# Luigi940260/orb-slam2-optimized

Measured on AMD Instinct MI355X. Metric: RANSAC hypotheses/sec (EPnP relocalization batch, 2k corrs x 64 candidates), higher is better.
Workload: dtype f64; 1 GPU; config 2 reloc_pnp: candidates x correspondences, iterate(300), exhaustive (40% inliers); candidates=64, candidates_per_gpu=64, correspondences=2000, hypotheses_per_candidate=300, params=SetRansacParameters(0.99,10,300,4,0.5,5.991)

## Files before the change

### orb-slam2-optimized_amd/csrc/kernels.hip

```cpp
#include <hip/hip_runtime.h>
#include <climits>

#ifndef RSC_REFINE_STAMPS
#define RSC_REFINE_STAMPS 0
#endif
namespace rsc {
__device__ uint64_t g_refine_stamps[64][24];
}
#ifndef RSC_SOLVE_STAMPS
#define RSC_SOLVE_STAMPS 0
#endif
namespace rsc {
__device__ uint64_t g_solve_stamps[3][4096][8];
}
#if RSC_SOLVE_STAMPS
#define RSC_JSVD_STAMP(k, j)                                                                           \
    do {                                                                                               \
        if (blockIdx.x < 4096 && (threadIdx.x & 63) == 0 && blockDim.x == 64) {                       \
            ::rsc::g_solve_stamps[2][blockIdx.x][j] = wall_clock64();                                  \
            ::rsc::g_solve_stamps[2][blockIdx.x][3] = (k);                                             \
        }                                                                                              \
    } while (0)
#define RSC_SOLVE_STAMP(st, k)                                                                         \
    do {                                                                                               \
        if (blockIdx.x < 4096 && (threadIdx.x & 63) == 0) ::rsc::g_solve_stamps[st][blockIdx.x][k] = wall_clock64(); \
    } while (0)
#endif
#include "rsc_core.h"
#include "rsc_epnp.h"
#include "rsc_sim3.h"
#if RSC_REFINE_STAMPS
#define RSC_EIG_PHASE(k)                                                                               \
    do {                                                                                               \
        if (blockIdx.x < 64 && threadIdx.x == 0) ::rsc::g_refine_stamps[blockIdx.x][8 + (k)] = wall_clock64(); \
    } while (0)
#endif
#include "rsc_quad.h"
#include "rsc_math.h"
#include "rsc_kernels.h"

namespace rsc {

template <int NS>
__global__ __launch_bounds__(64) void pnp_eig_group_kernel(const DevPnP* __restrict__ probs,
                                                          const LaunchProb* __restrict__ lps,
                                                          const int2* __restrict__ wg_table,
                                                          const uint32_t* __restrict__ rng_T,
                                                          double* __restrict__ stage, int32_t* __restrict__ samples) {
    __shared__ __attribute__((aligned(16))) double smem[kEigHyps * kQuadRegion];
    pnp_eig_group_body<NS, 99, kEigLanes, kEigHyps>(probs, lps, wg_table, rng_T, stage, samples, smem);
}

template <int NS>
__global__ __launch_bounds__(128 * kSplitUnits) __attribute__((amdgpu_waves_per_eu(2))) void pnp_eig_split_kernel(
    const DevPnP* __restrict__ probs, const LaunchProb* __restrict__ lps, const int2* __restrict__ wg_table,
    int nwg_table, const uint32_t* __restrict__ rng_T, double* __restrict__ stage, int32_t* __restrict__ samples,
    unsigned* fault) {
    __shared__ __attribute__((aligned(16))) double smem[kSplitHyps * kQuadRegion];
    __shared__ __attribute__((aligned(16))) double dsub[kSplitHyps * kSplitDsub];
    __shared__ int pub[kSplitUnits], ack[kSplitUnits];
    pnp_eig_split_body<NS>(probs, lps, wg_table, nwg_table, rng_T, stage, samples, smem, dsub, pub, ack, fault);
}

template <int NS>
__global__ __launch_bounds__(64) void pnp_betas_kernel(const DevPnP* __restrict__ probs,
                                                       const LaunchProb* __restrict__ lps,
                                                       const int2* __restrict__ wg_table, int ngroups,
                                                       const double* __restrict__ stage,
                                                       const int32_t* __restrict__ samples,
                                                       double* __restrict__ berr, float* __restrict__ bpose,
                                                       size_t hcap, int hb) {
    __shared__ __attribute__((aligned(16))) double smem[kBetasWaveSmemDoubles];
    pnp_betas_wave_body<NS>(probs, lps, wg_table, ngroups, hb, stage, samples, berr, bpose, hcap, smem);
}

typedef float rsc_f2 __attribute__((ext_vector_type(2)));
__device__ __forceinline__ void pnp_inlier2(const float (&R)[9], const float (&t)[3], double fx, double fy, double cx,
                                            double cy, rsc_f2 X, rsc_f2 Y, rsc_f2 Z, rsc_f2 u, rsc_f2 v, rsc_f2 maxErr,
                                            bool& in0, bool& in1, bool& ok) {
    const rsc_f2 Xc = (R[0] * X + (R[1] * Y + R[2] * Z)) + t[0];
    const rsc_f2 Yc = (R[3] * X + (R[4] * Y + R[5] * Z)) + t[1];
    const rsc_f2 Zc = (R[6] * X + (R[7] * Y + R[8] * Z)) + t[2];
    const rsc_f2 r0 = {__builtin_amdgcn_rcpf(Zc.x), __builtin_amdgcn_rcpf(Zc.y)};
    const rsc_f2 e = __builtin_elementwise_fma(-Zc, r0, (rsc_f2){1.0f, 1.0f});
    const rsc_f2 iz = __builtin_elementwise_fma(e, r0, r0);
    const float a0 = fabsf(Zc.x), a1 = fabsf(Zc.y);
    ok = ok & (a0 >= 0x1p-126f) & (a0 <= 0x1p125f) & (a1 >= 0x1p-126f) & (a1 <= 0x1p125f);
    const rsc_f2 ue = {(float)(cx + fx * (double)Xc.x * (double)iz.x), (float)(cx + fx * (double)Xc.y * (double)iz.y)};
    const rsc_f2 ve = {(float)(cy + fy * (double)Yc.x * (double)iz.x), (float)(cy + fy * (double)Yc.y * (double)iz.y)};
    const rsc_f2 du = ue - u, dv = ve - v;
    const rsc_f2 e2 = du * du + dv * dv;
    in0 = e2.x < maxErr.x;
    in1 = e2.y < maxErr.y;
}

template <int PPT>
__global__ __launch_bounds__(256) void pnp_scan_kernel(const DevPnP* __restrict__ probs,
                                                       const LaunchProb* __restrict__ lps,
                                                       const int4* __restrict__ wg_table,
                                                       const double* __restrict__ berr,
                                                       const float* __restrict__ bpose, size_t hcap,
                                                       float* __restrict__ poses,
                                                       int32_t* __restrict__ counts,
                                                       int32_t* __restrict__ counts_dev,
                                                       uint64_t* __restrict__ masks, int mask_words,
                                                       int32_t* __restrict__ qual) {
    constexpr int B = PPT <= 8 ? 64 : 512 / PPT;
    __shared__ int wave_cnt[4][B];
    __shared__ uint64_t mbuf[B][4][PPT];
    const int tid = threadIdx.x, lane = tid & 63, wave = tid >> 6;
    const int4 wt = wg_table[blockIdx.x];
    const LaunchProb& lp = lps[wt.x];
    const DevPnP& P = probs[lp.prob];
    const double fx = P.fx, fy = P.fy, cx = P.cx, cy = P.cy;
    const size_t rec0 = (size_t)(lp.out0 + wt.y);
    double e0 = 0.0, e1 = 0.0, e2 = 0.0;
    if (lane < wt.z) {
        e0 = berr[rec0 + lane];
        e1 = berr[hcap + rec0 + lane];
        e2 = berr[2 * hcap + rec0 + lane];
    }
    float X[PPT], Y[PPT], Z[PPT], U[PPT], V[PPT], E[PPT];
    RSC_UNROLL for (int s = 0; s < PPT; ++s) {
        const int i = s * 256 + tid;
        if (i < P.n) {
            const float4 p = P.pts[i];
            const float2 q = P.uv[i];
            X[s] = p.x; Y[s] = p.y; Z[s] = p.z; E[s] = p.w * P.th2; U[s] = q.x; V[s] = q.y;
        } else {
            X[s] = 0.f; Y[s] = 0.f; Z[s] = 1.f; E[s] = -1.f; U[s] = 0.f; V[s] = 0.f;
        }
    }
    int best = 0;
    {
        double be = e0;
        if (e1 < be) { be = e1; best = 1; }
        if (e2 < be) { be = e2; best = 2; }
    }
    const uint64_t pick1 = __ballot(best == 1), pick2 = __ballot(best == 2);
    auto pose_of = [&](int j) {
        const size_t apx = (size_t)((pick1 >> j) & 1u) + 2 * (size_t)((pick2 >> j) & 1u);
        return bpose + (apx * hcap + rec0 + (size_t)j) * 12;
    };
    for (int w = tid; w < wt.z * 12; w += 256) {
        const int hj = w / 12, k = w - 12 * hj;
        poses[(rec0 + hj) * 12 + k] = pose_of(hj)[k];
    }
    const float* pp = pose_of(0);
    float Rn[9], tn[3];
    RSC_UNROLL for (int k = 0; k < 9; ++k) Rn[k] = pp[k];
    RSC_UNROLL for (int k = 0; k < 3; ++k) tn[k] = pp[9 + k];
    for (int j = 0; j < wt.z; ++j) {
        float R[9], t[3];
        RSC_UNROLL for (int k = 0; k < 9; ++k) R[k] = Rn[k];
        RSC_UNROLL for (int k = 0; k < 3; ++k) t[k] = tn[k];
        if (j + 1 < wt.z) {
            pp = pose_of(j + 1);
            RSC_UNROLL for (int k = 0; k < 9; ++k) Rn[k] = pp[k];
            RSC_UNROLL for (int k = 0; k < 3; ++k) tn[k] = pp[9 + k];
        }
        uint64_t b[PPT];
        if constexpr (PPT >= 2) {
            bool ok = true;
            RSC_UNROLL for (int s = 0; s < PPT; s += 2) {
                bool i0, i1;
                pnp_inlier2(R, t, fx, fy, cx, cy, (rsc_f2){X[s], X[s + 1]}, (rsc_f2){Y[s], Y[s + 1]},
                            (rsc_f2){Z[s], Z[s + 1]}, (rsc_f2){U[s], U[s + 1]}, (rsc_f2){V[s], V[s + 1]},
                            (rsc_f2){E[s], E[s + 1]}, i0, i1, ok);
                b[s] = __ballot(i0);
                b[s + 1] = __ballot(i1);
            }
            if (__builtin_expect(__any(!ok), 0)) {
                RSC_UNROLL for (int s = 0; s < PPT; ++s)
                    b[s] = __ballot(pnp_inlier(R, t, fx, fy, cx, cy, X[s], Y[s], Z[s], U[s], V[s], E[s]));
            }
        } else {
            RSC_UNROLL for (int s = 0; s < PPT; ++s)
                b[s] = __ballot(pnp_inlier(R, t, fx, fy, cx, cy, X[s], Y[s], Z[s], U[s], V[s], E[s]));
        }
        int cnt = 0;
        uint64_t mine = 0;
        RSC_UNROLL for (int s = 0; s < PPT; ++s) {
            cnt += __popcll(b[s]);
            mine = (lane == s) ? b[s] : mine;
        }
        const int jb = j % B;
        if (lane < PPT) mbuf[jb][wave][lane] = mine;
        if (lane == 0) wave_cnt[wave][jb] = cnt;
        if (jb == B - 1 || j == wt.z - 1) {
            __syncthreads();
            const int base = j - jb;
            if (tid <= jb) {
                const int c = wave_cnt[0][tid] + wave_cnt[1][tid] + wave_cnt[2][tid] + wave_cnt[3][tid];
                counts[lp.out0 + wt.y + base + tid] = c;
                if (counts_dev) counts_dev[lp.out0 + wt.y + base + tid] = c;
                if (c >= lp.min_inliers) qual[wt.x] = 1;
                wave_cnt[0][tid] = c;
            }
            __syncthreads();
            if (masks) {
                for (int w = tid; w < (jb + 1) * 4 * PPT; w += 256) {
                    const int hb = w / (4 * PPT), r = w - hb * (4 * PPT), s = r >> 2, wv = r & 3;
                    if (wave_cnt[0][hb] >= lp.min_inliers)
                        masks[(size_t)(lp.out0 + wt.y + base + hb) * mask_words + r] = mbuf[hb][wv][s];
                }
            }
            __syncthreads();
        }
    }
}

__device__ __forceinline__ void wave_lds_sync() {
    __builtin_amdgcn_fence(__ATOMIC_RELEASE, "wavefront");
    __builtin_amdgcn_wave_barrier();
    __builtin_amdgcn_fence(__ATOMIC_ACQUIRE, "wavefront");
}

__device__ __forceinline__ double fold_col(double s, const double* col, int r, int m) {
    for (; r + 16 <= m; r += 16) {
        double v[16];
        RSC_UNROLL for (int k = 0; k < 16; ++k) v[k] = col[r + k];
        RSC_UNROLL for (int k = 0; k < 16; ++k) s = s + v[k];
    }
    for (; r < m; ++r) s = s + col[r];
    return s;
}

constexpr int kFoldStride = 65;

#ifndef RSC_REFINE_EIG_LANES
#define RSC_REFINE_EIG_LANES 4
#endif
constexpr int kRefineEigLanes = RSC_REFINE_EIG_LANES;
#ifndef RSC_REFINE_SPLIT
#define RSC_REFINE_SPLIT 0
#endif
#ifndef RSC_REFINE_LANE_ROWS
#define RSC_REFINE_LANE_ROWS 1
#endif
constexpr bool kRefineLaneRows = RSC_REFINE_LANE_ROWS != 0;
#ifndef RSC_FOLD_PIPE
#define RSC_FOLD_PIPE 1
#endif
#ifndef RSC_MTM_PIPELINE
#define RSC_MTM_PIPELINE 1
#endif
static_assert(kRefineEigLanes == 2 || kRefineEigLanes == 4, "refine eigen group: pair or quad");

template <int NS>
__global__ __launch_bounds__(256) void pnp_eig_rows_kernel(const DevPnP* __restrict__ probs,
                                                           const LaunchProb* __restrict__ lps,
                                                           const int2* __restrict__ wg_table,
                                                           const uint32_t* __restrict__ rng_T,
                                                           double* __restrict__ stage, int32_t* __restrict__ samples) {
    __shared__ __attribute__((aligned(16))) double smem[kEigHyps * kRowsRegion];
    pnp_eig_rows_body<NS, kRefineEigLanes>(probs, lps, wg_table, rng_T, stage, samples, smem, [] { wave_lds_sync(); });
}

#if RSC_FOLD_PIPE
constexpr int kFoldStride2 = 66;
template <int K, class Load, class Term>
__device__ __forceinline__ double wave_ordered_sum(int count, double* buf, bool from_zero, Load&& load, Term&& term) {
    constexpr int CS = kFoldStride2;
    const int lane = threadIdx.x & 63;
    const int colk = lane < K ? lane : K - 1;
    double s = 0.0;
    if (count <= 0) return s;
    const int nb = (count + 63) / 64;
    auto put = [&](int b, const auto& v) {
        double t[K];
        term(min(b * 64 + lane, count - 1), v, t);
        double* dst = buf + (b & 1) * (K * CS) + lane;
        RSC_UNROLL for (int k = 0; k < K; ++k) dst[k * CS] = t[k];
    };
    auto v = load(min(lane, count - 1));
    put(0, v);
    v = load(min(64 + lane, count - 1));
    wave_lds_sync();
    for (int b = 0; b < nb; ++b) {
        const double* c = buf + (b & 1) * (K * CS) + colk * CS;
        const bool steady = (b + 1 < nb) & (b * 64 + 64 <= count) & ((b > 0) | from_zero);
        if (steady) {
            const auto vn = v;
            v = load(min((b + 2) * 64 + lane, count - 1));
            put(b + 1, vn);
            const double2* c2 = reinterpret_cast<const double2*>(c);
            RSC_UNROLL for (int g = 0; g < 4; ++g) {
                double2 x[8];
                RSC_UNROLL for (int q = 0; q < 8; ++q) x[q] = c2[8 * g + q];
                RSC_UNROLL for (int q = 0; q < 8; ++q) {
                    s = s + x[q].x;
                    s = s + x[q].y;
                }
            }
        } else {
            if (b + 1 < nb) {
                const auto vn = v;
                v = load(min((b + 2) * 64 + lane, count - 1));
                put(b + 1, vn);
            }
            const int m = min(64, count - b * 64);
            int r = 0;
            if (b == 0 && !from_zero) {
                s = c[0];
                r = 1;
            }
            s = fold_col(s, c, r, m);
        }
        wave_lds_sync();
    }
    return s;
}
#else
template <int K, class Load, class Term>
__device__ __forceinline__ double wave_ordered_sum(int count, double* buf, bool from_zero, Load&& load, Term&& term) {
    const int lane = threadIdx.x & 63;
    double s = 0.0;
    auto next = load(min(lane, max(count - 1, 0)));
    for (int base = 0; base < count; base += 64) {
        const int i = base + lane;
        const auto v = next;
        if (i < count) {
            double t[K];
            term(i, v, t);
            RSC_UNROLL for (int k = 0; k < K; ++k) buf[k * kFoldStride + lane] = t[k];
        }
        if (base + 64 < count) next = load(min(i + 64, count - 1));
        wave_lds_sync();
        if (lane < K) {
            const int m = min(64, count - base);
            const double* col = buf + lane * kFoldStride;
            int r = 0;
            if (base == 0 && !from_zero) { s = col[0]; r = 1; }
            s = fold_col(s, col, r, m);
        }
        wave_lds_sync();
    }
    return s;
}

#endif

struct RefRow {
    double a[4], p[3], u[2];
};

__device__ __forceinline__ void refine_stamp(int slot) {
    if (RSC_REFINE_STAMPS && blockIdx.x < 64 && threadIdx.x == 0) g_refine_stamps[blockIdx.x][slot] = wall_clock64();
}
__device__ __forceinline__ void refine_wave_stamp(int wave, int j) {
    if (RSC_REFINE_STAMPS && blockIdx.x < 64 && (threadIdx.x & 63) == 0)
        g_refine_stamps[blockIdx.x][12 + 4 * wave + j] = wall_clock64();
}

__device__ __forceinline__ void pnp_refine_body(const DevPnP* __restrict__ probs, const RefineJob& J, unsigned* fault) {
    __shared__ __attribute__((aligned(16))) double slab[kSlabDoubles];
#if RSC_FOLD_PIPE
    __shared__ __attribute__((aligned(16))) double wbuf[4][2 * 9 * kFoldStride2];
#else
    __shared__ __attribute__((aligned(16))) double wbuf[4][kFoldStride * 9];
#endif
    __shared__ int prefix[129];
    __shared__ double cen_sh[3], cws_sh[12], cci_sh[9];
    __shared__ double res_sh[3][13];
    __shared__ float pose_sh[12];
    __shared__ int cnt_sh[4];
    const int tid = threadIdx.x, lane = tid & 63, wave = tid >> 6;
    const DevPnP& P = probs[J.prob];
    const int n = P.n;
    const int nwords = (n + 63) / 64;
    double* buf = wbuf[wave];

    refine_stamp(0);
    if (J.adopt_mask)
        for (int wd = tid; wd < nwords; wd += 256) J.adopt_mask[wd] = J.best_mask[wd];
    if (J.adopt_pose && tid < 12) J.out_best_pose[tid] = J.adopt_pose[tid];
    const uint64_t tail = (n & 63) ? (1ull << (n & 63)) - 1ull : ~0ull;
    auto best_word = [&](int wd) {
        const uint64_t m = J.best_mask[wd];
        return wd == nwords - 1 ? (m & tail) : m;
    };
    if (tid < 64) {
        int carry = 0;
        for (int w0 = 0; w0 < nwords; w0 += 64) {
            const int wd = w0 + lane;
            const int c = wd < nwords ? __popcll(best_word(wd)) : 0;
            int x = c;
            RSC_UNROLL for (int off = 1; off < 64; off <<= 1) {
                const int y = __shfl_up(x, off);
                if (lane >= off) x += y;
            }
            if (wd < nwords) prefix[wd] = carry + x - c;
            carry += __shfl(x, 63);
        }
        if (lane == 0) prefix[nwords] = carry;
    }
    __syncthreads();
    const int nr = prefix[nwords];
    for (int i = tid; i < n; i += 256) {
        const int wd = i >> 6, b = i & 63;
        const uint64_t m = best_word(wd);
        if ((m >> b) & 1ull) {
            const int r = prefix[wd] + __popcll(m & ((1ull << b) - 1ull));
            const float4 p = P.pts[i];
            const float2 q = P.uv[i];
            P.pws[3 * r + 0] = p.x; P.pws[3 * r + 1] = p.y; P.pws[3 * r + 2] = p.z;
            P.us[2 * r + 0] = q.x; P.us[2 * r + 1] = q.y;
        }
    }
    const int rows = J.rows_after;
    __syncthreads();
    refine_stamp(1);

    const double* __restrict__ pws = P.pws;
    const double* __restrict__ us = P.us;
    double* __restrict__ als = P.als;
    RowStore st{nr, rows, P.pws, P.us, P.als};
    const Intrinsics K{(double)P.fx, (double)P.fy, (double)P.cx, (double)P.cy};
    LaneMat S{slab, 1};
    if (wave == 0) {
        auto ld_p = [&](int i) { return RefRow{{0, 0, 0, 0}, {pws[3 * i], pws[3 * i + 1], pws[3 * i + 2]}, {0, 0}}; };
        const double cs = wave_ordered_sum<3>(rows, buf, false, ld_p, [&](int, const RefRow& v, double (&t)[3]) {
            t[0] = v.p[0]; t[1] = v.p[1]; t[2] = v.p[2];
        });
        if (lane < 3) cen_sh[lane] = cs / nr;
        wave_lds_sync();
        const double c0 = cen_sh[0], c1 = cen_sh[1], c2 = cen_sh[2];
        const double as = wave_ordered_sum<6>(nr, buf, false, ld_p, [&](int, const RefRow& v, double (&t)[6]) {
            const double d0 = v.p[0] - c0, d1 = v.p[1] - c1, d2 = v.p[2] - c2;
            t[0] = d0 * d0; t[1] = d0 * d1; t[2] = d0 * d2; t[3] = d1 * d1; t[4] = d1 * d2; t[5] = d2 * d2;
        });
        if (lane < 6) buf[lane] = as;
        wave_lds_sync();
        {
            double cws[4][3];
            cws[0][0] = c0; cws[0][1] = c1; cws[0][2] = c2;
            const double A[3][3] = {{buf[0], buf[1], buf[2]}, {buf[1], buf[3], buf[4]}, {buf[2], buf[4], buf[5]}};
            double V[3][3], w[3];
            sym_eig_reg<double, 3>(A, V, w);
            RSC_UNROLL for (int i = 0; i < 3; ++i) {
                double k = sqrt(w[i] / nr);
                RSC_UNROLL for (int c = 0; c < 3; ++c) cws[i + 1][c] = cws[0][c] + k * V[c][i];
            }
            double CC[3][3], CCi[3][3];
            RSC_UNROLL for (int i = 0; i < 3; ++i)
                RSC_UNROLL for (int j = 1; j < 4; ++j) CC[i][j - 1] = cws[j][i] - cws[0][i];
            inverse3(CC, CCi);
            RSC_UNROLL for (int i = 0; i < 4; ++i)
                RSC_UNROLL for (int c = 0; c < 3; ++c) cws_sh[3 * i + c] = cws[i][c];
            RSC_UNROLL for (int i = 0; i < 3; ++i)
                RSC_UNROLL for (int c = 0; c < 3; ++c) cci_sh[3 * i + c] = CCi[i][c];
        }
    }
    __syncthreads();
    for (int i = tid; i < nr; i += 256) {
        const double d0 = pws[3 * i] - cws_sh[0], d1 = pws[3 * i + 1] - cws_sh[1], d2 = pws[3 * i + 2] - cws_sh[2];
        const double a1 = ered3(cci_sh[0] * d0, cci_sh[1] * d1, cci_sh[2] * d2);
        const double a2 = ered3(cci_sh[3] * d0, cci_sh[4] * d1, cci_sh[5] * d2);
        const double a3 = ered3(cci_sh[6] * d0, cci_sh[7] * d1, cci_sh[8] * d2);
        als[4 * i + 1] = a1;
        als[4 * i + 2] = a2;
        als[4 * i + 3] = a3;
        als[4 * i + 0] = 1.0 - a1 - a2 - a3;
    }
    __threadfence_block();
    __syncthreads();
    refine_stamp(2);
#if RSC_MTM_PIPELINE
    {
        constexpr int kPairs = 128, kMtmRS = 2 * kPairs + 2;
        __shared__ __attribute__((aligned(16))) double mtm_buf[2][12 * kMtmRS];
        const bool folder = wave < 2 && lane < 39;
        int a = 0, b = wave * 39 + lane;
        while (b > a) { b -= a + 1; ++a; }
        const int nchunks = (nr + kPairs - 1) / kPairs;
        auto stage = [&](int c, int t0, int nt) {
            const int i0 = c * kPairs, m = min(kPairs, nr - i0);
            double* dst = mtm_buf[c & 1];
            for (int t = t0; t < m; t += nt) {
                const int i = i0 + t;
                const double al4[4] = {als[4 * i], als[4 * i + 1], als[4 * i + 2], als[4 * i + 3]};
                const double u0 = us[2 * i], u1 = us[2 * i + 1];
                RSC_UNROLL for (int j = 0; j < 4; ++j) {
                    *reinterpret_cast<double2*>(dst + (3 * j) * kMtmRS + 2 * t) = double2{al4[j] * K.fx, 0.0};
                    *reinterpret_cast<double2*>(dst + (3 * j + 1) * kMtmRS + 2 * t) = double2{0.0, al4[j] * K.fy};
                    *reinterpret_cast<double2*>(dst + (3 * j + 2) * kMtmRS + 2 * t) =
                        double2{al4[j] * (K.cx - u0), al4[j] * (K.cy - u1)};
                }
            }
        };
        if (nchunks > 0) stage(0, tid, 256);
        __syncthreads();
        double s = 0.0;
        for (int c = 0; c < nchunks; ++c) {
            if (wave >= 2 && c + 1 < nchunks) stage(c + 1, tid - 128, 128);
            if (folder) {
                const double* Ma = mtm_buf[c & 1] + a * kMtmRS;
                const double* Mb = mtm_buf[c & 1] + b * kMtmRS;
                const int m = 2 * min(kPairs, nr - c * kPairs);
                int r = 0;
                if (c == 0) {
                    s = Ma[0] * Mb[0];
                    s = s + Ma[1] * Mb[1];
                    r = 2;
                }
                if (r + 8 <= m) {
                    double p[8];
                    RSC_UNROLL for (int k = 0; k < 4; ++k) {
                        const double2 x = *reinterpret_cast<const double2*>(Ma + r + 2 * k);
                        const double2 y = *reinterpret_cast<const double2*>(Mb + r + 2 * k);
                        p[2 * k] = x.x * y.x;
                        p[2 * k + 1] = x.y * y.y;
                    }
                    for (r += 8; r + 8 <= m; r += 8) {
                        double2 x[4], y[4];
                        RSC_UNROLL for (int k = 0; k < 4; ++k) {
                            x[k] = *reinterpret_cast<const double2*>(Ma + r + 2 * k);
                            y[k] = *reinterpret_cast<const double2*>(Mb + r + 2 * k);
                        }
                        RSC_UNROLL for (int k = 0; k < 8; ++k) s = s + p[k];
                        RSC_UNROLL for (int k = 0; k < 4; ++k) {
                            p[2 * k] = x[k].x * y[k].x;
                            p[2 * k + 1] = x[k].y * y[k].y;
                        }
                    }
                    RSC_UNROLL for (int k = 0; k < 8; ++k) s = s + p[k];
                }
                for (; r < m; ++r) s = s + Ma[r] * Mb[r];
            }
            __syncthreads();
        }
        if (folder) S.at(a, b) = s;
    }
#else
    {
        constexpr int kPairs = (4 * kFoldStride * 9) / 24;
        __shared__ __attribute__((aligned(16))) double mtm_stage2[kPairs * 24];
        auto chunk_buf = [&](int c) { return (c & 1) ? mtm_stage2 : &wbuf[0][0]; };
        const bool folder = wave < 2 && lane < 39;
        int a = 0, b = wave * 39 + lane;
        while (b > a) { b -= a + 1; ++a; }
        const int nchunks = (nr + kPairs - 1) / kPairs;
        auto stage = [&](int c, int t0, int nt) {
            const int i0 = c * kPairs, m = min(kPairs, nr - i0);
            double* dst = chunk_buf(c);
            for (int t = t0; t < m; t += nt) {
                const int i = i0 + t;
                const double al4[4] = {als[4 * i], als[4 * i + 1], als[4 * i + 2], als[4 * i + 3]};
                const double u0 = us[2 * i], u1 = us[2 * i + 1];
                double* ev = dst + 24 * t;
                double* od = ev + 12;
                RSC_UNROLL for (int j = 0; j < 4; ++j) {
                    ev[3 * j] = al4[j] * K.fx;
                    ev[3 * j + 1] = 0.0;
                    ev[3 * j + 2] = al4[j] * (K.cx - u0);
                    od[3 * j] = 0.0;
                    od[3 * j + 1] = al4[j] * K.fy;
                    od[3 * j + 2] = al4[j] * (K.cy - u1);
                }
            }
        };
        if (nchunks > 0) stage(0, tid, 256);
        __syncthreads();
        double s = 0.0;
        for (int c = 0; c < nchunks; ++c) {
            if (wave >= 2 && c + 1 < nchunks) stage(c + 1, tid - 128, 128);
            if (folder) {
                const double* M = chunk_buf(c);
                const int m = 2 * min(kPairs, nr - c * kPairs);
                int r = 0;
                if (c == 0) {
                    s = M[a] * M[b];
                    r = 1;
                }
                for (; r + 8 <= m; r += 8) {
                    double x[8], y[8];
                    RSC_UNROLL for (int k = 0; k < 8; ++k) { x[k] = M[(r + k) * 12 + a]; y[k] = M[(r + k) * 12 + b]; }
                    RSC_UNROLL for (int k = 0; k < 8; ++k) s = s + x[k] * y[k];
                }
                for (; r < m; ++r) s = s + M[r * 12 + a] * M[r * 12 + b];
            }
            __syncthreads();
        }
        if (folder) S.at(a, b) = s;
    }
#endif
    __syncthreads();
    refine_stamp(3);
#if RSC_REFINE_SPLIT
    {
        __shared__ int rpub, rack;
        if (tid == 0) { rpub = 0; rack = 0; }
        if (wave == 0) refine_eig12_bc<kRefineEigLanes>(slab, &wbuf[0][0], lane, [] { wave_lds_sync(); });
        __syncthreads();
        if (RSC_REFINE_STAMPS && blockIdx.x < 64 && tid == 0)
            g_refine_stamps[blockIdx.x][8] = g_refine_stamps[blockIdx.x][9] = wall_clock64();
        if (wave == 0) {
            if (lane == 0) refine_eig12_chase(&wbuf[0][0], &wbuf[1][0], &rpub, &rack, fault);
            if (RSC_REFINE_STAMPS && blockIdx.x < 64 && tid == 0) g_refine_stamps[blockIdx.x][10] = wall_clock64();
        } else if (wave == 1 && lane < 12) {
            double ev[4];
            refine_eig12_rows(slab, &wbuf[1][0], &rpub, &rack, fault, lane, ev);
            RSC_UNROLL for (int c = 0; c < 4; ++c) slab[lane * 12 + c] = ev[c];
        }
        __syncthreads();
        if (RSC_REFINE_STAMPS && blockIdx.x < 64 && tid == 0) g_refine_stamps[blockIdx.x][11] = wall_clock64();
    }
#else
    if (wave == 0) {
        double ev[4];
        rows_eig12_ev4<kRefineEigLanes>(slab, &wbuf[0][0], lane, [] { wave_lds_sync(); }, ev);
        if (lane < 12) RSC_UNROLL for (int c = 0; c < 4; ++c) slab[lane * 12 + c] = ev[c];
    }
    __syncthreads();
#endif
    if (wave == 0) {
        compute_L_6x10(SlabView{S});
        auto d2 = [&](int a, int b) {
            double x = cws_sh[3 * a] - cws_sh[3 * b], y = cws_sh[3 * a + 1] - cws_sh[3 * b + 1],
                   z = cws_sh[3 * a + 2] - cws_sh[3 * b + 2];
            return ered3(x * x, y * y, z * z);
        };
        const SlabView SV{S};
        SV.rho(0) = d2(0, 1); SV.rho(1) = d2(0, 2); SV.rho(2) = d2(0, 3);
        SV.rho(3) = d2(1, 2); SV.rho(4) = d2(1, 3); SV.rho(5) = d2(2, 3);
    }
    __syncthreads();
    refine_stamp(4);
    if (wave < 3) {
        const SlabView SV{S};
        __shared__ double ccs_sh[3][12];
        {
            double betas[4] = {0.0, 0.0, 0.0, 0.0};
            if (wave == 0) find_betas<1, SlabView, kRefineLaneRows>(SV, betas);
            else if (wave == 1) find_betas<2, SlabView, kRefineLaneRows>(SV, betas);
            else find_betas<3, SlabView, kRefineLaneRows>(SV, betas);
            gauss_newton(SV, betas);
            double ccs[4][3];
            ccs_with_sign(st, SV, betas, ccs);
            RSC_UNROLL for (int i = 0; i < 4; ++i)
                RSC_UNROLL for (int c = 0; c < 3; ++c) ccs_sh[wave][3 * i + c] = ccs[i][c];
        }
        wave_lds_sync();
        refine_wave_stamp(wave, 0);
        double ccs[4][3];
        RSC_UNROLL for (int i = 0; i < 4; ++i)
            RSC_UNROLL for (int c = 0; c < 3; ++c) ccs[i][c] = ccs_sh[wave][3 * i + c];
        const double pw0[3] = {cws_sh[0], cws_sh[1], cws_sh[2]};
        auto ld_a = [&](int i) {
            return RefRow{{als[4 * i], als[4 * i + 1], als[4 * i + 2], als[4 * i + 3]}, {0, 0, 0}, {0, 0}};
        };
        const double ps = wave_ordered_sum<3>(rows, buf, false, ld_a, [&](int, const RefRow& v, double (&t)[3]) {
            RSC_UNROLL for (int c = 0; c < 3; ++c) t[c] = pcs_of(v.a, ccs, c);
        });
        __shared__ double pc0_sh[3][3];
        if (lane < 3) pc0_sh[wave][lane] = ps / nr;
        wave_lds_sync();
        refine_wave_stamp(wave, 1);
        const double pc0[3] = {pc0_sh[wave][0], pc0_sh[wave][1], pc0_sh[wave][2]};
        auto ld_ap = [&](int i) {
            return RefRow{{als[4 * i], als[4 * i + 1], als[4 * i + 2], als[4 * i + 3]},
                          {pws[3 * i], pws[3 * i + 1], pws[3 * i + 2]}, {0, 0}};
        };
        const double ms = wave_ordered_sum<9>(nr, buf, true, ld_ap, [&](int, const RefRow& v, double (&t)[9]) {
            double a[3], b[3];
            RSC_UNROLL for (int c = 0; c < 3; ++c) { a[c] = pcs_of(v.a, ccs, c) - pc0[c]; b[c] = v.p[c] - pw0[c]; }
            RSC_UNROLL for (int r = 0; r < 3; ++r)
                RSC_UNROLL for (int c = 0; c < 3; ++c) t[3 * r + c] = a[r] * b[c];
        });
        __shared__ double m_sh[3][9];
        if (lane < 9) m_sh[wave][lane] = ms;
        wave_lds_sync();
        __shared__ double rt_sh[3][12];
        {
            double M[3][3], R[3][3], t[3];
            RSC_UNROLL for (int r = 0; r < 3; ++r)
                RSC_UNROLL for (int c = 0; c < 3; ++c) M[r][c] = m_sh[wave][3 * r + c];
            horn_from_M(M, pc0, pw0, R, t);
            RSC_UNROLL for (int k = 0; k < 9; ++k) rt_sh[wave][k] = R[k / 3][k % 3];
            RSC_UNROLL for (int k = 0; k < 3; ++k) rt_sh[wave][9 + k] = t[k];
        }
        wave_lds_sync();
        refine_wave_stamp(wave, 2);
        double R[3][3], t[3];
        RSC_UNROLL for (int k = 0; k < 9; ++k) R[k / 3][k % 3] = rt_sh[wave][k];
        RSC_UNROLL for (int k = 0; k < 3; ++k) t[k] = rt_sh[wave][9 + k];
        auto ld_pu = [&](int i) {
            return RefRow{{0, 0, 0, 0}, {pws[3 * i], pws[3 * i + 1], pws[3 * i + 2]}, {us[2 * i], us[2 * i + 1]}};
        };
        const double es = wave_ordered_sum<1>(nr, buf, true, ld_pu, [&](int, const RefRow& v, double (&tt)[1]) {
            tt[0] = reproj_term(R, t, K, v.p[0], v.p[1], v.p[2], v.u[0], v.u[1]);
        });
        if (lane == 0) {
            RSC_UNROLL for (int k = 0; k < 12; ++k) res_sh[wave][k] = rt_sh[wave][k];
            res_sh[wave][12] = es / nr;
        }
        refine_wave_stamp(wave, 3);
    }
    __syncthreads();
    refine_stamp(5);
    if (tid == 0) {
        int b = 0;
        if (res_sh[1][12] < res_sh[b][12]) b = 1;
        if (res_sh[2][12] < res_sh[b][12]) b = 2;
        RSC_UNROLL for (int k = 0; k < 12; ++k) pose_sh[k] = (float)res_sh[b][k];
    }
    __syncthreads();
    float R[9], t[3];
    RSC_UNROLL for (int k = 0; k < 9; ++k) R[k] = pose_sh[k];
    RSC_UNROLL for (int k = 0; k < 3; ++k) t[k] = pose_sh[9 + k];
    int cnt = 0;
    const double fx = P.fx, fy = P.fy, cx = P.cx, cy = P.cy;
    const int mask_words_out = J.out_words;
    for (int base = 0; base < mask_words_out * 64; base += 256) {
        const int i = base + tid;
        bool inl = false;
        if (i < n) {
            const float4 p = P.pts[i];
            const float2 q = P.uv[i];
            inl = pnp_inlier(R, t, fx, fy, cx, cy, p.x, p.y, p.z, q.x, q.y, p.w * P.th2);
        }
        const uint64_t b = __ballot(inl);
        cnt += __popcll(b);
        if (lane == 0 && (base / 64 + wave) < mask_words_out) J.out_mask[base / 64 + wave] = b;
    }
    if (lane == 0) cnt_sh[wave] = cnt;
    __syncthreads();
    refine_stamp(6);
    if (tid == 0) {
        *J.out_count = cnt_sh[0] + cnt_sh[1] + cnt_sh[2] + cnt_sh[3];
        RSC_UNROLL for (int k = 0; k < 12; ++k) J.out_pose[k] = pose_sh[k];
    }
}

__global__ __launch_bounds__(256) void pnp_refine_kernel(const DevPnP* __restrict__ probs,
                                                         const RefineJob* __restrict__ jobs, unsigned* fault) {
    const RefineJob J = jobs[blockIdx.x];
    pnp_refine_body(probs, J, fault);
}

__global__ __launch_bounds__(256) void pnp_select_refine_kernel(const DevPnP* __restrict__ probs,
                                                                const RefineSel* __restrict__ sels,
                                                                const int32_t* __restrict__ counts,
                                                                uint64_t* __restrict__ masks, int mask_words,
                                                                const float* __restrict__ poses,
                                                                RefineSelOut* __restrict__ out, unsigned* fault) {
    __shared__ int k_sh;
    const RefineSel S = sels[blockIdx.x];
    const int tid = threadIdx.x;
    if (tid < 64) {
        int k = -1;
        for (int base = 0; base < S.H && k < 0; base += 64) {
            const int idx = base + tid;
            const bool q = idx < S.H && counts[S.out0 + idx] >= S.min_inliers;
            const uint64_t b = __ballot(q);
            if (b) k = base + __ffsll((unsigned long long)b) - 1;
        }
        if (tid == 0) k_sh = k;
    }
    __syncthreads();
    const int k = k_sh;
    RefineSelOut& o = out[blockIdx.x];
    if (k < 0) {
        if (tid == 0) o.k = -1;
        return;
    }
    const size_t rec = (size_t)(S.out0 + k);
    const int c = counts[rec];
    const bool adopt = c > S.best0;
    const int nr = adopt ? c : S.best0;
    RefineJob J;
    J.prob = S.prob;
    J.rows_after = max(S.rows0, nr);
    J.best_mask = adopt ? masks + rec * mask_words : S.best;
    J.adopt_mask = adopt ? S.best : nullptr;
    J.adopt_pose = adopt ? poses + rec * 12 : nullptr;
    J.out_best_pose = o.best_pose;
    J.out_pose = o.pose;
    J.out_count = &o.count;
    J.out_mask = S.refined;
    J.out_words = S.words;
    if (tid == 0) {
        o.k = k;
        o.adopt = adopt ? 1 : 0;
        o.rows_after = J.rows_after;
    }
    pnp_refine_body(probs, J, fault);
}

__global__ __launch_bounds__(64) void sim3_solve_kernel(const DevSim3* __restrict__ probs,
                                                        const LaunchProb* __restrict__ lps,
                                                        const int2* __restrict__ wg_table,
                                                        const uint32_t* __restrict__ rng_T,
                                                        float* __restrict__ poses, int32_t* __restrict__ samples) {
    const int lane = threadIdx.x;
    const int2 wt = wg_table[blockIdx.x];
    const LaunchProb& lp = lps[wt.x];
    const int h = wt.y + lane;
    if (h >= lp.H) return;
    const DevSim3& P = probs[lp.prob];
    uint32_t w[31];
    RSC_UNROLL for (int j = 0; j < 31; ++j) w[j] = lp.window[j];
    uint32_t words[3];
    RSC_UNROLL for (int d = 0; d < 3; ++d) words[d] = rng_word(rng_T, w, lp.g0 + h * 3 + d);
    int idx[3];
    swap_remove_sample<3>(words, 3, P.n, idx);
    float P1[3][3], P2[3][3];
    RSC_UNROLL for (int i = 0; i < 3; ++i) {
        const float4 a = P.x1[idx[i]];
        const float4 b = P.x2[idx[i]];
        P1[0][i] = a.x; P1[1][i] = a.y; P1[2][i] = a.z;
        P2[0][i] = b.x; P2[1][i] = b.y; P2[2][i] = b.z;
    }
    Sim3Pose T;
    sim3_compute(P1, P2, T);
    float* out = poses + (size_t)(lp.out0 + h) * 24;
    RSC_UNROLL for (int k = 0; k < 9; ++k) out[k] = T.R12[k];
    RSC_UNROLL for (int k = 0; k < 3; ++k) out[9 + k] = T.t12[k];
    RSC_UNROLL for (int k = 0; k < 9; ++k) out[12 + k] = T.R21[k];
    RSC_UNROLL for (int k = 0; k < 3; ++k) out[21 + k] = T.t21[k];
    if (samples) {
        RSC_UNROLL for (int i = 0; i < 3; ++i) samples[(size_t)(lp.out0 + h) * 8 + i] = idx[i];
    }
}

template <int PPT>
__global__ __launch_bounds__(256) void sim3_scan_kernel(const DevSim3* __restrict__ probs,
                                                        const LaunchProb* __restrict__ lps,
                                                        const int4* __restrict__ wg_table,
                                                        const float* __restrict__ poses,
                                                        int32_t* __restrict__ counts,
                                                        int32_t* __restrict__ counts_dev,
                                                        uint64_t* __restrict__ masks, int mask_words) {
    __shared__ int wave_cnt[4][64];
    const int tid = threadIdx.x, lane = tid & 63, wave = tid >> 6;
    const int4 wt = wg_table[blockIdx.x];
    const LaunchProb& lp = lps[wt.x];
    const DevSim3& P = probs[lp.prob];
    const float K1[4] = {P.K1[0], P.K1[1], P.K1[2], P.K1[3]};
    const float K2[4] = {P.K2[0], P.K2[1], P.K2[2], P.K2[3]};
    float A[PPT][3], B[PPT][3], p1u[PPT], p1v[PPT], p2u[PPT], p2v[PPT], e1[PPT], e2[PPT];
    RSC_UNROLL for (int s = 0; s < PPT; ++s) {
        const int i = s * 256 + tid;
        if (i < P.n) {
            const float4 a = P.x1[i], b = P.x2[i], pp = P.pim[i];
            A[s][0] = a.x; A[s][1] = a.y; A[s][2] = a.z; e1[s] = a.w;
            B[s][0] = b.x; B[s][1] = b.y; B[s][2] = b.z; e2[s] = b.w;
            p1u[s] = pp.x; p1v[s] = pp.y; p2u[s] = pp.z; p2v[s] = pp.w;
        } else {
            A[s][0] = A[s][1] = 0.f; A[s][2] = 1.f; B[s][0] = B[s][1] = 0.f; B[s][2] = 1.f;
            e1[s] = e2[s] = -1.f; p1u[s] = p1v[s] = p2u[s] = p2v[s] = 0.f;
        }
    }
    for (int j = 0; j < wt.z; ++j) {
        const int h = wt.y + j;
        const float* pp = poses + (size_t)(lp.out0 + h) * 24;
        Sim3Pose T;
        RSC_UNROLL for (int k = 0; k < 9; ++k) { T.R12[k] = pp[k]; T.R21[k] = pp[12 + k]; }
        RSC_UNROLL for (int k = 0; k < 3; ++k) { T.t12[k] = pp[9 + k]; T.t21[k] = pp[21 + k]; }
        uint64_t b[PPT];
        RSC_UNROLL for (int s = 0; s < PPT; ++s)
            b[s] = __ballot(sim3_inlier(T, K1, K2, A[s], B[s], p1u[s], p1v[s], p2u[s], p2v[s], e1[s], e2[s]));
        int cnt = 0;
        uint64_t mine = 0;
        RSC_UNROLL for (int s = 0; s < PPT; ++s) {
            cnt += __popcll(b[s]);
            mine = (lane == s) ? b[s] : mine;
        }
        if (masks && lane < PPT) masks[(size_t)(lp.out0 + h) * mask_words + lane * 4 + wave] = mine;
        if (lane == 0) wave_cnt[wave][j & 63] = cnt;
        if ((j & 63) == 63 || j == wt.z - 1) {
            __syncthreads();
            const int base = j & ~63;
            if (tid <= (j & 63)) {
                const int c = wave_cnt[0][tid] + wave_cnt[1][tid] + wave_cnt[2][tid] + wave_cnt[3][tid];
                counts[lp.out0 + wt.y + base + tid] = c;
                if (counts_dev) counts_dev[lp.out0 + wt.y + base + tid] = c;
            }
            __syncthreads();
        }
    }
}

__global__ void gather_records_kernel(const float* __restrict__ src, int stride, int take,
                                      const int32_t* __restrict__ idx, int n, float* __restrict__ dst) {
    const int t = blockIdx.x * blockDim.x + threadIdx.x;
    if (t >= n * take) return;
    const int q = t / take, e = t - q * take;
    dst[t] = src[(size_t)idx[q] * stride + e];
}

__global__ __launch_bounds__(256) void sim3_pick_kernel(const LaunchProb* __restrict__ lps,
                                                        const int32_t* __restrict__ counts,
                                                        const float* __restrict__ poses, float* __restrict__ pick) {
    constexpr int T = 256, PER = kPickMaxH / T;
    __shared__ int pre[T];
    __shared__ int ret_k, keep_k;
    const int tid = threadIdx.x;
    const LaunchProb& lp = lps[blockIdx.x];
    const int H = lp.H;
    const int per = (H + T - 1) / T;
    int c[PER];
    int mx = INT_MIN;
    RSC_UNROLL for (int u = 0; u < PER; ++u) {
        const int k = tid * per + u;
        c[u] = (u < per && k < H) ? counts[lp.out0 + k] : INT_MIN;
        mx = max(mx, c[u]);
    }
    pre[tid] = mx;
    if (tid == 0) { ret_k = INT_MAX; keep_k = -1; }
    __syncthreads();
    for (int d = 1; d < T; d <<= 1) {
        const int v = (tid >= d) ? pre[tid - d] : INT_MIN;
        __syncthreads();
        pre[tid] = max(pre[tid], v);
        __syncthreads();
    }
    int run = max(lp.best0, tid > 0 ? pre[tid - 1] : INT_MIN);
    int my_ret = INT_MAX;
    RSC_UNROLL for (int u = 0; u < PER; ++u) {
        const int k = tid * per + u;
        if (u < per && k < H && c[u] >= run) {
            run = c[u];
            if (c[u] > lp.min_inliers) my_ret = min(my_ret, k);
        }
    }
    atomicMin(&ret_k, my_ret);
    __syncthreads();
    const int r = ret_k;
    run = max(lp.best0, tid > 0 ? pre[tid - 1] : INT_MIN);
    int my_keep = -1;
    RSC_UNROLL for (int u = 0; u < PER; ++u) {
        const int k = tid * per + u;
        if (u < per && k < H && k <= r && c[u] >= run) {
            run = c[u];
            my_keep = k;
        }
    }
    atomicMax(&keep_k, my_keep);
    __syncthreads();
    const int k = keep_k;
    float* o = pick + (size_t)blockIdx.x * 16;
    if (tid == 0) reinterpret_cast<int32_t*>(o)[0] = k;
    if (k >= 0 && tid < 12) o[1 + tid] = poses[(size_t)(lp.out0 + k) * 24 + tid];
}

hipError_t launch_sim3_pick(int count, const LaunchProb* lps, const int32_t* counts, const float* poses,
                            float* pick, hipStream_t st) {
    if (count <= 0) return hipSuccess;
    sim3_pick_kernel<<<count, 256, 0, st>>>(lps, counts, poses, pick);
    return hipGetLastError();
}

hipError_t launch_gather_records(const float* src, int stride, int take, const int32_t* idx, int n, float* dst,
                                 hipStream_t st) {
    if (n <= 0) return hipSuccess;
    gather_records_kernel<<<(n * take + 255) / 256, 256, 0, st>>>(src, stride, take, idx, n, dst);
    return hipGetLastError();
}

__global__ void rng_stream_kernel(const uint32_t* __restrict__ T, Window31 w, int g0, int n, int32_t* __restrict__ out) {
    const int i = blockIdx.x * blockDim.x + threadIdx.x;
    if (i >= n) return;
    uint32_t ww[31];
    RSC_UNROLL for (int j = 0; j < 31; ++j) ww[j] = w.w[j];
    out[i] = (int32_t)(rng_word(T, ww, g0 + i) >> 1);
}

template <int N>
static hipError_t launch_eig_rows(int nwgE, const int2* wgtE, const DevPnP* probs, const LaunchProb* lps,
                                  const uint32_t* T, double* stage, int32_t* samples, hipStream_t st) {
    if constexpr (kEigHyps == 4 * kRowsGroups) {
        pnp_eig_rows_kernel<N><<<nwgE, 256, 0, st>>>(probs, lps, wgtE, T, stage, samples);
        return hipSuccess;
    } else {
        return hipErrorInvalidValue;
    }
}

hipError_t launch_pnp_solve_split(int ns, int nwgE, const int2* wgtE, int nwgB, const int2* wgtB,
                                  const DevPnP* probs, const LaunchProb* lps, const uint32_t* T, double* stage,
                                  int32_t* samples, const BetasScratch& bs, hipStream_t st,
                                  hipEvent_t eig_begin, hipEvent_t eig_end, bool eig_rows, bool eig_split,
                                  unsigned* fault, int betas_hb) {
    if (ns < 4 || ns > 6 || betas_hb < 1 || betas_hb > kBetasHyps) return hipErrorInvalidValue;
    if (eig_split && !eig_rows && !fault) return hipErrorInvalidValue;
    if (eig_begin) (void)hipEventRecord(eig_begin, st);
    switch (ns) {
#define RSC_CASE(N)                                                                                   \
    case N:                                                                                           \
        if (eig_rows) {                                                                               \
            const hipError_t e = launch_eig_rows<N>(nwgE, wgtE, probs, lps, T, stage, samples, st);   \
            if (e != hipSuccess) return e;                                                            \
        } else if (eig_split)                                                                         \
            pnp_eig_split_kernel<N><<<(nwgE + kSplitUnits - 1) / kSplitUnits, 128 * kSplitUnits, 0, st>>>( \
                probs, lps, wgtE, nwgE, T, stage, samples, fault);                                    \
        else                                                                                          \
            pnp_eig_group_kernel<N><<<nwgE, 64, 0, st>>>(probs, lps, wgtE, T, stage, samples);        \
        if (eig_end) (void)hipEventRecord(eig_end, st);                                               \
        pnp_betas_kernel<N><<<3 * nwgB, 64, 0, st>>>(probs, lps, wgtB, nwgB, stage, samples,          \
                                                     bs.err, bs.pose, bs.hcap, betas_hb);             \
        break;
        RSC_CASE(4) RSC_CASE(5) RSC_CASE(6)
#undef RSC_CASE
        default: return hipErrorInvalidValue;
    }
    return hipGetLastError();
}

__global__ __launch_bounds__(256) void selftest_math_kernel(int fn, const double* __restrict__ x, int n,
                                                            double* __restrict__ out) {
    const int i = blockIdx.x * 256 + threadIdx.x;
    if (i >= n) return;
    const double v = x[i];
    double r;
    switch (fn) {
        case 0: r = dm::sin(v); break;
        case 1: r = dm::cos(v); break;
        case 2: r = dm::acos(v); break;
        case 3: r = dm::cbrt(v); break;
        case 4: r = dm::log(v); break;
        case 5: r = (double)dm::logf((float)v); break;
        case 6: r = sqrt_unit(v); break;
        case 7: r = recip_unit(v); break;
        case 11: r = dm::pow_1_3(v); break;
        case 12: r = dm::pow_3_2(v); break;
        case 13: {
            const float z = (float)v;
            const float r0 = __builtin_amdgcn_rcpf(z);
            r = (double)__builtin_fmaf(__builtin_fmaf(-z, r0, 1.0f), r0, r0);
            break;
        }

        default: {
            double c, s;
            make_givens(v, x[(i + n / 2) % n], c, s);
            r = fn == 8 ? c : s;
            break;
        }
    }
    out[i] = r;
}

__global__ __launch_bounds__(256) void selftest_qr_kernel(const double* __restrict__ x, int nrec,
                                                          double* __restrict__ out) {
    const int r = blockIdx.x * 256 + threadIdx.x;
    if (r >= nrec) return;
    const double* in = x + 34 * (size_t)r;
    double A[6][4], b[6], X[4];
    RSC_UNROLL for (int i = 0; i < 6; ++i) {
        RSC_UNROLL for (int j = 0; j < 4; ++j) A[i][j] = in[4 * i + j];
        b[i] = in[24 + i];
    }
    RSC_UNROLL for (int j = 0; j < 4; ++j) X[j] = in[30 + j];
    const bool ok = qr_solve_6x4(A, b, X);
    double* o = out + 34 * (size_t)r;
    RSC_UNROLL for (int j = 0; j < 4; ++j) o[j] = X[j];
    o[4] = ok ? 1.0 : 0.0;
    for (int j = 5; j < 34; ++j) o[j] = 0.0;
}

__global__ __launch_bounds__(256) void upload16_kernel(const uint4* __restrict__ src, uint4* __restrict__ dst, size_t n16) {
    const size_t i = (size_t)blockIdx.x * 256 + threadIdx.x;
    if (i < n16) dst[i] = src[i];
}

__global__ __launch_bounds__(256) void copy_bytes_kernel(const uint8_t* __restrict__ src, uint8_t* __restrict__ dst,
                                                         size_t n, int unit) {
    const size_t b = ((size_t)blockIdx.x * 256 + threadIdx.x) * 16;
    if (b >= n) return;
    if (b + 16 <= n && unit == 16) {
        *reinterpret_cast<uint4*>(dst + b) = *reinterpret_cast<const uint4*>(src + b);
    } else if (b + 16 <= n && unit == 4) {
        RSC_UNROLL for (int k = 0; k < 16; k += 4)
            *reinterpret_cast<uint32_t*>(dst + b + k) = *reinterpret_cast<const uint32_t*>(src + b + k);
    } else {
        const size_t e = (b + 16 < n) ? b + 16 : n;
        for (size_t k = b; k < e; ++k) dst[k] = src[k];
    }
}

hipError_t launch_copy_bytes(const void* src, void* dst, size_t n, hipStream_t st) {
    if (n == 0) return hipSuccess;
    const uintptr_t a = reinterpret_cast<uintptr_t>(src) | reinterpret_cast<uintptr_t>(dst);
    const int unit = (a % 16 == 0) ? 16 : (a % 4 == 0 ? 4 : 1);
    const unsigned blocks = (unsigned)((n + 16 * 256 - 1) / (16 * 256));
    copy_bytes_kernel<<<blocks, 256, 0, st>>>(static_cast<const uint8_t*>(src), static_cast<uint8_t*>(dst), n, unit);
    return hipGetLastError();
}

__global__ __launch_bounds__(64) void signal_kernel(uint32_t* flag, uint32_t v) {
    if (threadIdx.x == 0) __hip_atomic_store(flag, v, __ATOMIC_RELEASE, __HIP_MEMORY_SCOPE_SYSTEM);
}

hipError_t launch_signal(uint32_t* host_flag, uint32_t value, hipStream_t st) {
    signal_kernel<<<1, 64, 0, st>>>(host_flag, value);
    return hipGetLastError();
}

hipError_t launch_upload16(const void* host_src, void* dev_dst, size_t n16, hipStream_t st) {
    if (n16 == 0) return hipSuccess;
    const unsigned blocks = (unsigned)((n16 + 255) / 256);
    upload16_kernel<<<blocks, 256, 0, st>>>(static_cast<const uint4*>(host_src), static_cast<uint4*>(dev_dst), n16);
    return hipGetLastError();
}

hipError_t launch_selftest_math(int fn, const double* x, int n, double* out, hipStream_t st) {
    if (fn < 0 || fn > 13 || n <= 0) return hipErrorInvalidValue;
    if (fn == 10) {
        if (n % 34) return hipErrorInvalidValue;
        const int nrec = n / 34;
        selftest_qr_kernel<<<(nrec + 255) / 256, 256, 0, st>>>(x, nrec, out);
        return hipGetLastError();
    }
    selftest_math_kernel<<<(n + 255) / 256, 256, 0, st>>>(fn, x, n, out);
    return hipGetLastError();
}

hipError_t launch_pnp_scan(int ppt, int nwg, const DevPnP* probs, const LaunchProb* lps, const int4* wgt,
                           const BetasScratch& bs, float* poses, int32_t* counts, int32_t* counts_dev, uint64_t* masks,
                           int mask_words, int32_t* qual, hipStream_t st) {
    switch (ppt) {
#define RSC_CASE(P) case P: pnp_scan_kernel<P><<<nwg, 256, 0, st>>>(probs, lps, wgt, bs.err, bs.pose, bs.hcap, poses, counts, counts_dev, masks, mask_words, qual); break;
        RSC_CASE(1) RSC_CASE(2) RSC_CASE(4) RSC_CASE(8) RSC_CASE(16) RSC_CASE(32)
#undef RSC_CASE
        default: return hipErrorInvalidValue;
    }
    return hipGetLastError();
}

hipError_t pnp_scan_occupancy(int ppt, int* wgs_per_cu) {
    switch (ppt) {
#define RSC_CASE(P) case P: return hipOccupancyMaxActiveBlocksPerMultiprocessor(wgs_per_cu, reinterpret_cast<const void*>(&pnp_scan_kernel<P>), 256, 0);
        RSC_CASE(1) RSC_CASE(2) RSC_CASE(4) RSC_CASE(8) RSC_CASE(16) RSC_CASE(32)
#undef RSC_CASE
        default: return hipErrorInvalidValue;
    }
}

hipError_t read_solve_stamps(uint64_t* out) {
    return hipMemcpyFromSymbol(out, HIP_SYMBOL(g_solve_stamps), sizeof(uint64_t) * 3 * 4096 * 8, 0, hipMemcpyDeviceToHost);
}

hipError_t read_refine_stamps(uint64_t* out) {
    return hipMemcpyFromSymbol(out, HIP_SYMBOL(g_refine_stamps), sizeof(uint64_t) * 64 * 24, 0, hipMemcpyDeviceToHost);
}

hipError_t launch_pnp_refine(int njobs, const DevPnP* probs, const RefineJob* jobs, unsigned* fault, hipStream_t st) {
    if (!fault) return hipErrorInvalidValue;
    pnp_refine_kernel<<<njobs, 256, 0, st>>>(probs, jobs, fault);
    return hipGetLastError();
}

hipError_t launch_pnp_select_refine(int nsel, const DevPnP* probs, const RefineSel* sels, const int32_t* counts,
                                    uint64_t* masks, int mask_words, const float* poses, RefineSelOut* out,
                                    unsigned* fault, hipStream_t st) {
    if (nsel <= 0) return hipSuccess;
    if (!fault) return hipErrorInvalidValue;
    pnp_select_refine_kernel<<<nsel, 256, 0, st>>>(probs, sels, counts, masks, mask_words, poses, out, fault);
    return hipGetLastError();
}

hipError_t launch_sim3_solve(int nwg, const DevSim3* probs, const LaunchProb* lps, const int2* wgt, const uint32_t* T,
                             float* poses, int32_t* samples, hipStream_t st) {
    sim3_solve_kernel<<<nwg, 64, 0, st>>>(probs, lps, wgt, T, poses, samples);
    return hipGetLastError();
}

hipError_t launch_sim3_scan(int ppt, int nwg, const DevSim3* probs, const LaunchProb* lps, const int4* wgt,
                            const float* poses, int32_t* counts, int32_t* counts_dev, uint64_t* masks, int mask_words,
                            hipStream_t st) {
    switch (ppt) {
#define RSC_CASE(P) case P: sim3_scan_kernel<P><<<nwg, 256, 0, st>>>(probs, lps, wgt, poses, counts, counts_dev, masks, mask_words); break;
        RSC_CASE(1) RSC_CASE(2) RSC_CASE(4) RSC_CASE(8) RSC_CASE(16) RSC_CASE(32)
#undef RSC_CASE
        default: return hipErrorInvalidValue;
    }
    return hipGetLastError();
}

hipError_t launch_rng_stream(const uint32_t* T, const uint32_t* window, int g0, int n, int32_t* out, hipStream_t st) {
    Window31 w;
    for (int j = 0; j < 31; ++j) w.w[j] = window[j];
    rng_stream_kernel<<<(n + 255) / 256, 256, 0, st>>>(T, w, g0, n, out);
    return hipGetLastError();
}

}
```

Baseline: 75.31 million hypotheses/s.

## Write inlier mask only for first qualifying hypothesis via recompute pass

```diff
diff --git a/orb-slam2-optimized_amd/csrc/kernels.hip b/orb-slam2-optimized_amd/csrc/kernels.hip
--- a/orb-slam2-optimized_amd/csrc/kernels.hip
+++ b/orb-slam2-optimized_amd/csrc/kernels.hip
@@ -107,7 +107,7 @@
                                                        int32_t* __restrict__ qual) {
     constexpr int B = PPT <= 8 ? 64 : 512 / PPT;
     __shared__ int wave_cnt[4][B];
-    __shared__ uint64_t mbuf[B][4][PPT];
+    __shared__ int first_sh;
     const int tid = threadIdx.x, lane = tid & 63, wave = tid >> 6;
     const int4 wt = wg_table[blockIdx.x];
     const LaunchProb& lp = lps[wt.x];
@@ -146,20 +146,7 @@
         const int hj = w / 12, k = w - 12 * hj;
         poses[(rec0 + hj) * 12 + k] = pose_of(hj)[k];
     }
-    const float* pp = pose_of(0);
-    float Rn[9], tn[3];
-    RSC_UNROLL for (int k = 0; k < 9; ++k) Rn[k] = pp[k];
-    RSC_UNROLL for (int k = 0; k < 3; ++k) tn[k] = pp[9 + k];
-    for (int j = 0; j < wt.z; ++j) {
-        float R[9], t[3];
-        RSC_UNROLL for (int k = 0; k < 9; ++k) R[k] = Rn[k];
-        RSC_UNROLL for (int k = 0; k < 3; ++k) t[k] = tn[k];
-        if (j + 1 < wt.z) {
-            pp = pose_of(j + 1);
-            RSC_UNROLL for (int k = 0; k < 9; ++k) Rn[k] = pp[k];
-            RSC_UNROLL for (int k = 0; k < 3; ++k) tn[k] = pp[9 + k];
-        }
-        uint64_t b[PPT];
+    auto ballots = [&](const float (&R)[9], const float (&t)[3], uint64_t (&b)[PPT]) {
         if constexpr (PPT >= 2) {
             bool ok = true;
             RSC_UNROLL for (int s = 0; s < PPT; s += 2) {
@@ -178,34 +165,60 @@
             RSC_UNROLL for (int s = 0; s < PPT; ++s)
                 b[s] = __ballot(pnp_inlier(R, t, fx, fy, cx, cy, X[s], Y[s], Z[s], U[s], V[s], E[s]));
         }
-        int cnt = 0;
-        uint64_t mine = 0;
-        RSC_UNROLL for (int s = 0; s < PPT; ++s) {
-            cnt += __popcll(b[s]);
-            mine = (lane == s) ? b[s] : mine;
-        }
-        const int jb = j % B;
-        if (lane < PPT) mbuf[jb][wave][lane] = mine;
-        if (lane == 0) wave_cnt[wave][jb] = cnt;
-        if (jb == B - 1 || j == wt.z - 1) {
-            __syncthreads();
-            const int base = j - jb;
-            if (tid <= jb) {
-                const int c = wave_cnt[0][tid] + wave_cnt[1][tid] + wave_cnt[2][tid] + wave_cnt[3][tid];
-                counts[lp.out0 + wt.y + base + tid] = c;
-                if (counts_dev) counts_dev[lp.out0 + wt.y + base + tid] = c;
-                if (c >= lp.min_inliers) qual[wt.x] = 1;
-                wave_cnt[0][tid] = c;
-            }
-            __syncthreads();
-            if (masks) {
-                for (int w = tid; w < (jb + 1) * 4 * PPT; w += 256) {
-                    const int hb = w / (4 * PPT), r = w - hb * (4 * PPT), s = r >> 2, wv = r & 3;
-                    if (wave_cnt[0][hb] >= lp.min_inliers)
-                        masks[(size_t)(lp.out0 + wt.y + base + hb) * mask_words + r] = mbuf[hb][wv][s];
+    };
+    uint64_t todo = wt.z >= 64 ? ~0ull : (1ull << wt.z) - 1;
+    int first = -1;
+    for (int pass = 0; pass < 2; ++pass) {
+        float Rn[9] = {}, tn[3] = {};
+        if (todo) {
+            const float* pp = pose_of(__ffsll((unsigned long long)todo) - 1);
+            RSC_UNROLL for (int k = 0; k < 9; ++k) Rn[k] = pp[k];
+            RSC_UNROLL for (int k = 0; k < 3; ++k) tn[k] = pp[9 + k];
+        }
+        while (todo) {
+            const int j = __ffsll((unsigned long long)todo) - 1;
+            todo &= todo - 1;
+            float R[9], t[3];
+            RSC_UNROLL for (int k = 0; k < 9; ++k) R[k] = Rn[k];
+            RSC_UNROLL for (int k = 0; k < 3; ++k) t[k] = tn[k];
+            if (todo) {
+                const float* pp = pose_of(__ffsll((unsigned long long)todo) - 1);
+                RSC_UNROLL for (int k = 0; k < 9; ++k) Rn[k] = pp[k];
+                RSC_UNROLL for (int k = 0; k < 3; ++k) tn[k] = pp[9 + k];
+            }
+            uint64_t b[PPT];
+            ballots(R, t, b);
+            if (pass == 1) {
+                if (lane == 0) {
+                    uint64_t* row = masks + (rec0 + (size_t)j) * mask_words;
+                    RSC_UNROLL for (int s = 0; s < PPT; ++s) row[4 * s + wave] = b[s];
                 }
-            }
-            __syncthreads();
+                continue;
+            }
+            int cnt = 0;
+            RSC_UNROLL for (int s = 0; s < PPT; ++s) cnt += __popcll(b[s]);
+            const int jb = j % B;
+            if (lane == 0) wave_cnt[wave][jb] = cnt;
+            if (jb == B - 1 || !todo) {
+                __syncthreads();
+                const int base = j - jb;
+                bool q = false;
+                if (tid <= jb) {
+                    const int c = wave_cnt[0][tid] + wave_cnt[1][tid] + wave_cnt[2][tid] + wave_cnt[3][tid];
+                    counts[lp.out0 + wt.y + base + tid] = c;
+                    if (counts_dev) counts_dev[lp.out0 + wt.y + base + tid] = c;
+                    q = c >= lp.min_inliers;
+                    if (q) qual[wt.x] = 1;
+                }
+                const uint64_t qb = __ballot(q);
+                if (first < 0 && qb) first = base + __ffsll((unsigned long long)qb) - 1;
+                if (tid == 0) first_sh = first;
+                __syncthreads();
+            }
+        }
+        if (pass == 0 && masks && wt.z > 0) {
+            const int f = __builtin_amdgcn_readfirstlane(first_sh);
+            if (f >= 0) todo = 1ull << f;
         }
     }
 }
```

Result: faster. 76.71 million hypotheses/s, median of 6 (+1.9%).
